# tczhangzhi/pytorch-distributed

Hardware: NVIDIA H100
Metric: ResNet-50 images/sec (device-timed, max over ranks) (higher is better)
Workload: dtype bf16; 1 GPU; model=resnet50, global_batch=256, image_size=224, parallelism=dp1, entry=distributed, comm=fused, nvls=False, channels_last=True, fused_bn=True, optimizer=fused, cuda_graph=True, l2_policy=inputs larger than L2 (4 x 38.5 MB bf16 batches + GBs of activations per step), overlap_optimizer=True, bucket_view=False, cudnn=deterministic

## Files before the change

### pytorch_distributed_b200/csrc/bindings.cpp

```cpp
#include <torch/extension.h>

#include "hvd_core.h"
#include "host.h"
#include "symm.h"

namespace py = pybind11;
using namespace ptd;

namespace {

at::Tensor arena_view(const std::shared_ptr<SymmArena>& a, int64_t rank, int64_t offset_bytes, int64_t numel, const std::string& dtype) {
  at::ScalarType st;
  if (dtype == "float32") st = at::kFloat;
  else if (dtype == "bfloat16") st = at::kBFloat16;
  else if (dtype == "float16") st = at::kHalf;
  else if (dtype == "int32") st = at::kInt;
  else if (dtype == "uint8") st = at::kByte;
  else throw std::runtime_error("unsupported arena view dtype " + dtype);
  const int64_t esz = (int64_t)c10::elementSize(st);
  TORCH_CHECK(offset_bytes >= 0 && offset_bytes + numel * esz <= a->bytes(), "arena view out of range");
  TORCH_CHECK(offset_bytes % esz == 0, "misaligned arena view");
  const int r = a->single_process() ? (int)rank : a->rank();
  void* p = reinterpret_cast<void*>(a->ptr(r) + offset_bytes);
  auto keep = a;
  return at::from_blob(p, {numel}, [keep](void*) {}, at::TensorOptions().dtype(st).device(at::kCUDA, (c10::DeviceIndex)a->device(r)));
}

}

PYBIND11_MODULE(TORCH_EXTENSION_NAME, m) {
  m.doc() = "pytorch_distributed_b200 native runtime (sm_90a)";
  m.attr("MAX_WORLD") = kMaxWorld;
  m.attr("MAX_BLOCKS") = kMaxBlocks;
  m.attr("MAX_CHANNELS") = kMaxChannels;
  m.attr("MAX_PTRS") = kMaxPtrs;
  m.attr("SIGNAL_PAD_BYTES") = (int64_t)sizeof(SignalPad);
  m.attr("SEG_BYTES") = (int64_t)sizeof(Seg);
  m.def("multicast_supported", &multicast_supported);

  py::class_<SymmArena, std::shared_ptr<SymmArena>>(m, "SymmArena")
      .def(py::init<int, int, int, int64_t>(), py::arg("device"), py::arg("rank"), py::arg("world"), py::arg("bytes"))
      .def_static("create_local", &SymmArena::create_local)
      .def_static("from_pointers", &SymmArena::from_pointers)
      .def("export_fd", &SymmArena::export_fd)
      .def("open_socket", &SymmArena::open_socket)
      .def("send_fd", &SymmArena::send_fd)
      .def("recv_fd", &SymmArena::recv_fd, py::call_guard<py::gil_scoped_release>())
      .def("map_peer", &SymmArena::map_peer)
      .def("mc_create", &SymmArena::mc_create)
      .def("mc_import", &SymmArena::mc_import)
      .def("mc_add_device", &SymmArena::mc_add_device)
      .def("mc_bind_and_map", &SymmArena::mc_bind_and_map)
      .def("disable_multicast", &SymmArena::disable_multicast)
      .def_property_readonly("rank", &SymmArena::rank)
      .def_property_readonly("world", &SymmArena::world)
      .def_property_readonly("bytes", &SymmArena::bytes)
      .def_property_readonly("mc_ptr", &SymmArena::mc_ptr)
      .def_property_readonly("multicast_candidate", &SymmArena::multicast_candidate)
      .def_property_readonly("has_multicast", &SymmArena::has_multicast)
      .def_property_readonly("mc_error", &SymmArena::mc_error)
      .def_property_readonly("single_process", &SymmArena::single_process)
      .def("ptr", &SymmArena::ptr)
      .def("device", &SymmArena::device, py::arg("r") = 0)
      .def("status", &SymmArena::status)
      .def("set_timeout_ms", &SymmArena::set_timeout_ms)
      .def("ll_seq_ptr", &SymmArena::ll_seq_ptr, py::arg("r") = 0)
      .def("view", [](std::shared_ptr<SymmArena> a, int64_t offset, int64_t numel, const std::string& dtype, int64_t rank) {
             return arena_view(a, rank, offset, numel, dtype);
           }, py::arg("offset_bytes"), py::arg("numel"), py::arg("dtype"), py::arg("rank") = 0)
      .def("launch_plan",
           [](std::shared_ptr<SymmArena> a, int channel, int as_rank, int kind, int wire_dtype, bool nvls, int grid, std::vector<at::Tensor> tensors,
              int64_t seg_begin_ptr, int64_t segs_ptr, int64_t data_off_bytes, int64_t block_elems, int64_t plan_calls_ptr, int64_t found_inf_ptr,
              double scale, bool writeback, int root, int flags, int64_t result_off_bytes) {
             launch_plan(a->ctx(channel, as_rank), kind, wire_dtype, nvls, grid, tensors, seg_begin_ptr, segs_ptr, data_off_bytes, block_elems,
                         plan_calls_ptr, found_inf_ptr, scale, writeback, root, flags, result_off_bytes);
           },
           py::arg("channel"), py::arg("as_rank"), py::arg("kind"), py::arg("wire_dtype"), py::arg("nvls"), py::arg("grid"), py::arg("tensors"),
           py::arg("seg_begin_ptr"), py::arg("segs_ptr"), py::arg("data_off_bytes"), py::arg("block_elems"), py::arg("plan_calls_ptr"),
           py::arg("found_inf_ptr"), py::arg("scale"), py::arg("writeback"), py::arg("root"), py::arg("flags") = 0,
           py::arg("result_off_bytes") = (int64_t)-1)
      .def("launch_barrier", [](std::shared_ptr<SymmArena> a, int channel) { launch_barrier(a->ctx(channel)); })
      .def("launch_metrics",
           [](std::shared_ptr<SymmArena> a, int channel, const at::Tensor& logits, const at::Tensor& target, c10::optional<at::Tensor> loss, at::Tensor out) {
             launch_metrics(a->ctx(channel), logits, target, loss, a->ll_seq_ptr(), out);
           })
      .def("launch_ll_allreduce", [](std::shared_ptr<SymmArena> a, int channel, const at::Tensor& in, at::Tensor out, double scale) {
        launch_ll_allreduce(a->ctx(channel), in, out, scale, a->ll_seq_ptr());
      });

  m.def("pack_pointers", &pack_pointers);
  m.def("fused_sgd_flat", &fused_sgd_flat, py::arg("grad"), py::arg("master"), py::arg("momentum"), py::arg("model_copy"), py::arg("hyper"),
        py::arg("found_inf"), py::arg("nesterov"), py::arg("first_step"));
  m.def("fused_sgd_multi", &fused_sgd_multi);
  m.def("multi_tensor_scale", &multi_tensor_scale);
  m.def("multi_tensor_axpby", &multi_tensor_axpby);
  m.def("amp_update_scale", &amp_update_scale);
  m.def("bn_act_forward", &bn_act_forward);
  m.def("bn_act_backward", &bn_act_backward);
  m.def("bn_act_backward2", &bn_act_backward2);
  m.def("stem_forward", &stem_forward);
  m.def("stem_forward_pre", &stem_forward_pre);
  m.def("stem_backward", &stem_backward);
  m.def("stem_im2col", &stem_im2col);
  m.def("conv1x1_bnstats", &conv1x1_bnstats);
  m.def("normalize_nhwc", &normalize_nhwc);
  m.def("resample_normalize", &resample_normalize, py::arg("arena"), py::arg("n"), py::arg("out_h"), py::arg("out_w"), py::arg("max_rows"),
        py::arg("a"), py::arg("b"), py::arg("out_dtype"), py::arg("channels_last"));
  m.def("p2p_copy_multi", &p2p_copy_multi);

  py::class_<FusionQueue, std::shared_ptr<FusionQueue>>(m, "FusionQueue")
      .def(py::init<int64_t, double, int64_t>(), py::arg("fusion_threshold_bytes"), py::arg("cycle_time_ms"), py::arg("cycle_bytes") = 0)
      .def("wait_idle", &FusionQueue::wait_idle, py::arg("timeout_ms"), py::call_guard<py::gil_scoped_release>())
      .def("wake", &FusionQueue::wake)
      .def("set_cycle_bytes", &FusionQueue::set_cycle_bytes)
      .def("cycle_bytes", &FusionQueue::cycle_bytes)
      .def("enable_timeline", &FusionQueue::enable_timeline)
      .def("timeline", &FusionQueue::timeline)
      .def("enqueue", &FusionQueue::enqueue, py::arg("name"), py::arg("nbytes"), py::arg("order_key"))
      .def("next_group", &FusionQueue::next_group, py::arg("timeout_ms"), py::call_guard<py::gil_scoped_release>())
      .def("flush", &FusionQueue::flush)
      .def("mark_done", &FusionQueue::mark_done)
      .def("wait", &FusionQueue::wait, py::arg("handle"), py::arg("timeout_ms"), py::call_guard<py::gil_scoped_release>())
      .def("pending", &FusionQueue::pending)
      .def("shutdown", &FusionQueue::shutdown)
      .def("stats", &FusionQueue::stats);
}
```

### pytorch_distributed_b200/csrc/gemm_bnstats.cu

```cuda
#include <ATen/cuda/CUDAContext.h>
#include <c10/cuda/CUDAGuard.h>
#include <cuda.h>
#include <torch/extension.h>

#include "common.cuh"
#include "host.h"

namespace ptd {

constexpr int kBlockM = 128;
constexpr int kBlockK = 64;
constexpr int kConsumerThreads = 256;
constexpr int kGemmThreads = kConsumerThreads + 32;

template <int BLOCK_N> struct GemmCfg {
  static constexpr int kStages = BLOCK_N == 256 ? 3 : 4;
  static constexpr int kABytes = kBlockM * kBlockK * 2;
  static constexpr int kBBytes = BLOCK_N * kBlockK * 2;
  static constexpr int kCBytes = kBlockM * BLOCK_N * 2;
  static constexpr int kStatFloats = 2 * 4 * 128;
  static constexpr int kSmem = 1024 + kStages * (kABytes + kBBytes) + kCBytes + kStatFloats * 4 + 2 * kStages * 8;
};

__device__ __forceinline__ uint32_t smem_u32(const void* p) { return (uint32_t)__cvta_generic_to_shared(p); }

__device__ __forceinline__ void mbar_init(uint64_t* bar, uint32_t count) {
  asm volatile("mbarrier.init.shared::cta.b64 [%0], %1;" ::"r"(smem_u32(bar)), "r"(count));
}
__device__ __forceinline__ void mbar_expect_tx(uint64_t* bar, uint32_t bytes) {
  asm volatile("mbarrier.arrive.expect_tx.shared::cta.b64 _, [%0], %1;" ::"r"(smem_u32(bar)), "r"(bytes) : "memory");
}
__device__ __forceinline__ void mbar_arrive(uint64_t* bar) {
  asm volatile("mbarrier.arrive.shared::cta.b64 _, [%0];" ::"r"(smem_u32(bar)) : "memory");
}
__device__ __forceinline__ void mbar_wait(uint64_t* bar, uint32_t parity) {
  const uint32_t addr = smem_u32(bar);
  uint32_t done, spins = 0;
  do {
    asm volatile("{\n\t.reg .pred p;\n\tmbarrier.try_wait.parity.shared::cta.b64 p, [%1], %2;\n\tselp.u32 %0, 1, 0, p;\n\t}"
                 : "=r"(done) : "r"(addr), "r"(parity) : "memory");
    if (!done && ++spins > (1u << 24)) __trap();
  } while (!done);
}
__device__ __forceinline__ void tma_load_2d(void* smem_dst, const CUtensorMap* map, uint64_t* bar, int c0, int c1) {
  asm volatile("cp.async.bulk.tensor.2d.shared::cluster.global.mbarrier::complete_tx::bytes [%0], [%1, {%3, %4}], [%2];"
               ::"r"(smem_u32(smem_dst)), "l"(map), "r"(smem_u32(bar)), "r"(c0), "r"(c1) : "memory");
}
__device__ __forceinline__ void named_barrier(int id, int threads) {
  asm volatile("bar.sync %0, %1;" ::"r"(id), "r"(threads) : "memory");
}

__device__ __forceinline__ uint64_t gmma_desc(const void* smem_tile) {
  const uint64_t addr = (uint64_t)(smem_u32(smem_tile) >> 4) & 0x3FFFull;
  return addr | (1ull << 16) | ((uint64_t)(1024 >> 4) << 32) | (1ull << 62);
}

#define PTD_F8(i) "+f"(d[i]), "+f"(d[i + 1]), "+f"(d[i + 2]), "+f"(d[i + 3]), "+f"(d[i + 4]), "+f"(d[i + 5]), "+f"(d[i + 6]), "+f"(d[i + 7])

__device__ __forceinline__ void wgmma_n64(float* d, uint64_t adesc, uint64_t bdesc, int accumulate) {
  asm volatile(
      "{\n\t.reg .pred p;\n\tsetp.ne.b32 p, %34, 0;\n\t"
      "wgmma.mma_async.sync.aligned.m64n64k16.f32.bf16.bf16 "
      "{%0, %1, %2, %3, %4, %5, %6, %7, %8, %9, %10, %11, %12, %13, %14, %15, "
      "%16, %17, %18, %19, %20, %21, %22, %23, %24, %25, %26, %27, %28, %29, %30, %31}, %32, %33, p, 1, 1, 0, 0;\n\t}"
      : PTD_F8(0), PTD_F8(8), PTD_F8(16), PTD_F8(24)
      : "l"(adesc), "l"(bdesc), "r"(accumulate));
}
__device__ __forceinline__ void wgmma_n128(float* d, uint64_t adesc, uint64_t bdesc, int accumulate) {
  asm volatile(
      "{\n\t.reg .pred p;\n\tsetp.ne.b32 p, %66, 0;\n\t"
      "wgmma.mma_async.sync.aligned.m64n128k16.f32.bf16.bf16 "
      "{%0, %1, %2, %3, %4, %5, %6, %7, %8, %9, %10, %11, %12, %13, %14, %15, "
      "%16, %17, %18, %19, %20, %21, %22, %23, %24, %25, %26, %27, %28, %29, %30, %31, "
      "%32, %33, %34, %35, %36, %37, %38, %39, %40, %41, %42, %43, %44, %45, %46, %47, "
      "%48, %49, %50, %51, %52, %53, %54, %55, %56, %57, %58, %59, %60, %61, %62, %63}, %64, %65, p, 1, 1, 0, 0;\n\t}"
      : PTD_F8(0), PTD_F8(8), PTD_F8(16), PTD_F8(24), PTD_F8(32), PTD_F8(40), PTD_F8(48), PTD_F8(56)
      : "l"(adesc), "l"(bdesc), "r"(accumulate));
}
#undef PTD_F8

template <int N> __device__ __forceinline__ void fence_regs(float (&d)[N]) {
#pragma unroll
  for (int i = 0; i < N; ++i) asm volatile("" : "+f"(d[i])::"memory");
}

template <int BLOCK_N>
__global__ void __launch_bounds__(kGemmThreads, 1) gemm_bnstats_kernel(const __grid_constant__ CUtensorMap tmap_a,
                                                                       const __grid_constant__ CUtensorMap tmap_b,
                                                                       const __grid_constant__ CUtensorMap tmap_c,
                                                                       float* __restrict__ part, int N, int K, int m_tiles,
                                                                       int n_tiles, int ctas_per_n) {
  using Cfg = GemmCfg<BLOCK_N>;
  constexpr int kStages = Cfg::kStages;
  constexpr int kInstN = BLOCK_N >= 128 ? 128 : 64;
  constexpr int kBoxes = BLOCK_N / 64;
  extern __shared__ uint8_t smem_raw[];
  uint8_t* smem = reinterpret_cast<uint8_t*>((reinterpret_cast<uintptr_t>(smem_raw) + 1023) & ~(uintptr_t)1023);
  uint8_t* smem_a = smem;
  uint8_t* smem_b = smem_a + kStages * Cfg::kABytes;
  uint8_t* smem_c = smem_b + kStages * Cfg::kBBytes;
  float* smem_stats = reinterpret_cast<float*>(smem_c + Cfg::kCBytes);
  uint64_t* full_bar = reinterpret_cast<uint64_t*>(smem_stats + Cfg::kStatFloats);
  uint64_t* empty_bar = full_bar + kStages;

  const int warp = threadIdx.x >> 5, lane = threadIdx.x & 31;
  const int n_tile = blockIdx.x % n_tiles;
  const int m_first = blockIdx.x / n_tiles;
  const int n0 = n_tile * BLOCK_N;
  const int num_kb = K / kBlockK;

  if (threadIdx.x == 0) {
    for (int s = 0; s < kStages; ++s) { mbar_init(&full_bar[s], 1); mbar_init(&empty_bar[s], kConsumerThreads / 32); }
    asm volatile("fence.mbarrier_init.release.cluster;" ::: "memory");
  }
  __syncthreads();

  if (warp == kConsumerThreads / 32) {
    if (lane == 0) {
      asm volatile("prefetch.tensormap [%0];" ::"l"(&tmap_a) : "memory");
      asm volatile("prefetch.tensormap [%0];" ::"l"(&tmap_b) : "memory");
      uint32_t it = 0;
      for (int mt = m_first; mt < m_tiles; mt += ctas_per_n) {
        for (int kb = 0; kb < num_kb; ++kb, ++it) {
          const int s = it % kStages;
          mbar_wait(&empty_bar[s], ((it / kStages) & 1) ^ 1);
          mbar_expect_tx(&full_bar[s], Cfg::kABytes + Cfg::kBBytes);
          tma_load_2d(smem_a + s * Cfg::kABytes, &tmap_a, &full_bar[s], kb * kBlockK, mt * kBlockM);
          tma_load_2d(smem_b + s * Cfg::kBBytes, &tmap_b, &full_bar[s], kb * kBlockK, n0);
        }
      }
    }
    return;
  }

  const int wg = warp >> 2, t = threadIdx.x & 127, w = warp & 3;
  uint8_t* stg = smem_c + wg * (Cfg::kCBytes / 2);
  float acc[BLOCK_N / 2] = {};
  const int r0 = 16 * w + (lane >> 2);
  constexpr int kPairs = BLOCK_N / 2, kParts = 128 / kPairs, kRows = 64 / kParts;
  const int p = t % kPairs, rpart = t / kPairs;
  const int p_box = p >> 5, p_gran = (p & 31) >> 2, p_byte = (p & 3) * 4;
  float s0 = 0.f, s1 = 0.f, q0 = 0.f, q1 = 0.f;

  uint32_t it = 0;
  for (int mt = m_first; mt < m_tiles; mt += ctas_per_n) {
    for (int kb = 0; kb < num_kb; ++kb, ++it) {
      const int s = it % kStages;
      mbar_wait(&full_bar[s], (it / kStages) & 1);
      const uint64_t adesc = gmma_desc(smem_a + s * Cfg::kABytes + wg * 64 * 128);
      const uint64_t bdesc = gmma_desc(smem_b + s * Cfg::kBBytes);
      fence_regs(acc);
      asm volatile("wgmma.fence.sync.aligned;" ::: "memory");
#pragma unroll
      for (int k = 0; k < kBlockK / 16; ++k) {
#pragma unroll
        for (int h = 0; h < BLOCK_N / kInstN; ++h) {
          if constexpr (kInstN == 128) wgmma_n128(acc + h * 64, adesc + 2 * k, bdesc + h * 8 * kInstN + 2 * k, (kb | k) != 0);
          else wgmma_n64(acc + h * 32, adesc + 2 * k, bdesc + h * 8 * kInstN + 2 * k, (kb | k) != 0);
        }
      }
      asm volatile("wgmma.commit_group.sync.aligned;" ::: "memory");
      asm volatile("wgmma.wait_group.sync.aligned 0;" ::: "memory");
      fence_regs(acc);
      if (lane == 0) mbar_arrive(&empty_bar[s]);
    }

    if (t == 0) asm volatile("cp.async.bulk.wait_group.read 0;" ::: "memory");
    named_barrier(1 + wg, 128);
#pragma unroll
    for (int j = 0; j < BLOCK_N / 8; ++j) {
      uint8_t* box = stg + (j >> 3) * 8192 + (lane & 3) * 4;
      const int g = j & 7;
      *reinterpret_cast<uint32_t*>(box + r0 * 128 + ((g ^ (r0 & 7)) << 4)) = Wire<__nv_bfloat16>::pack2(acc[4 * j], acc[4 * j + 1]);
      *reinterpret_cast<uint32_t*>(box + (r0 + 8) * 128 + ((g ^ (r0 & 7)) << 4)) =
          Wire<__nv_bfloat16>::pack2(acc[4 * j + 2], acc[4 * j + 3]);
    }
    asm volatile("fence.proxy.async.shared::cta;" ::: "memory");
    named_barrier(1 + wg, 128);
    if (t == 0) {
#pragma unroll
      for (int b = 0; b < kBoxes; ++b)
        asm volatile("cp.async.bulk.tensor.2d.global.shared::cta.bulk_group [%0, {%2, %3}], [%1];"
                     ::"l"(&tmap_c), "r"(smem_u32(stg + b * 8192)), "r"(n0 + b * 64), "r"(mt * kBlockM + wg * 64) : "memory");
      asm volatile("cp.async.bulk.commit_group;" ::: "memory");
    }
    const uint8_t* src = stg + p_box * 8192 + p_byte;
#pragma unroll 8
    for (int r = rpart * kRows; r < rpart * kRows + kRows; ++r) {
      const float2 f = Wire<__nv_bfloat16>::unpack2(*reinterpret_cast<const uint32_t*>(src + r * 128 + ((p_gran ^ (r & 7)) << 4)));
      s0 += f.x; q0 += f.x * f.x;
      s1 += f.y; q1 += f.y * f.y;
    }
  }
  if (t == 0) asm volatile("cp.async.bulk.wait_group 0;" ::: "memory");
  float* my = smem_stats + wg * 4 * 128 + t;
  my[0] = s0; my[128] = s1; my[256] = q0; my[384] = q1;
  named_barrier(3, kConsumerThreads);
  for (int i = threadIdx.x; i < 2 * BLOCK_N; i += kConsumerThreads) {
    const int half = i >= BLOCK_N, col = i - half * BLOCK_N;
    const int pair = col >> 1, which = half * 2 + (col & 1);
    float v = 0.f;
    for (int w2 = 0; w2 < 2; ++w2)
      for (int pt = 0; pt < kParts; ++pt) v += smem_stats[w2 * 4 * 128 + which * 128 + pt * kPairs + pair];
    part[(size_t)m_first * 2 * N + half * N + n0 + col] = v;
  }
}

typedef CUresult (*EncodeTiledFn)(CUtensorMap*, CUtensorMapDataType, cuuint32_t, void*, const cuuint64_t*, const cuuint64_t*, const cuuint32_t*,
                                  const cuuint32_t*, CUtensorMapInterleave, CUtensorMapSwizzle, CUtensorMapL2promotion, CUtensorMapFloatOOBfill);

static EncodeTiledFn encode_fn() {
  static EncodeTiledFn fn = nullptr;
  if (!fn) {
    void* p = nullptr;
    cudaDriverEntryPointQueryResult q;
    TORCH_CHECK(cudaGetDriverEntryPoint("cuTensorMapEncodeTiled", &p, cudaEnableDefault, &q) == cudaSuccess && p, "cuTensorMapEncodeTiled not found");
    fn = reinterpret_cast<EncodeTiledFn>(p);
  }
  return fn;
}

static CUtensorMap make_map(const void* ptr, int64_t rows, int64_t cols, int box_rows, CUtensorMapL2promotion promo) {
  CUtensorMap m;
  cuuint64_t dims[2] = {(cuuint64_t)cols, (cuuint64_t)rows};
  cuuint64_t strides[1] = {(cuuint64_t)cols * 2};
  cuuint32_t box[2] = {(cuuint32_t)kBlockK, (cuuint32_t)box_rows};
  cuuint32_t estr[2] = {1, 1};
  CUresult r = encode_fn()(&m, CU_TENSOR_MAP_DATA_TYPE_BFLOAT16, 2, const_cast<void*>(ptr), dims, strides, box, estr, CU_TENSOR_MAP_INTERLEAVE_NONE,
                           CU_TENSOR_MAP_SWIZZLE_128B, promo, CU_TENSOR_MAP_FLOAT_OOB_FILL_NONE);
  TORCH_CHECK(r == CUDA_SUCCESS, "cuTensorMapEncodeTiled failed: ", (int)r);
  return m;
}

template <int BLOCK_N>
static void launch_gemm(const at::Tensor& a, const at::Tensor& b, at::Tensor& c, at::Tensor& gsum, int M, int N, int K) {
  constexpr int smem = GemmCfg<BLOCK_N>::kSmem;
  static bool configured[64] = {};
  const int dev = a.get_device();
  if (!configured[dev & 63]) {
    C10_CUDA_CHECK(cudaFuncSetAttribute(gemm_bnstats_kernel<BLOCK_N>, cudaFuncAttributeMaxDynamicSharedMemorySize, smem));
    configured[dev & 63] = true;
  }
  const CUtensorMap ma = make_map(a.data_ptr(), M, K, kBlockM, CU_TENSOR_MAP_L2_PROMOTION_L2_256B);
  const CUtensorMap mb = make_map(b.data_ptr(), N, K, BLOCK_N, CU_TENSOR_MAP_L2_PROMOTION_L2_256B);
  const CUtensorMap mc = make_map(c.data_ptr(), M, N, 64, CU_TENSOR_MAP_L2_PROMOTION_NONE);
  const int m_tiles = (M + kBlockM - 1) / kBlockM, n_tiles = N / BLOCK_N;
  const int sms = at::cuda::getCurrentDeviceProperties()->multiProcessorCount;
  const int ctas_per_n = std::max(1, std::min(m_tiles, sms / n_tiles));
  const int grid = ctas_per_n * n_tiles;
  cudaStream_t st = at::cuda::getCurrentCUDAStream();
  at::Tensor part = at::empty({ctas_per_n, 2 * N}, gsum.options());
  gemm_bnstats_kernel<BLOCK_N><<<grid, kGemmThreads, smem, st>>>(ma, mb, mc, part.data_ptr<float>(), N, K, m_tiles, n_tiles, ctas_per_n);
  C10_CUDA_KERNEL_LAUNCH_CHECK();
  combine_partials(part.data_ptr<float>(), ctas_per_n, 2 * N, gsum.data_ptr<float>(), st);
}

at::Tensor conv1x1_bnstats(const at::Tensor& x, const at::Tensor& weight, at::Tensor gsum) {
  TORCH_CHECK(x.is_cuda() && x.dim() == 4 && x.scalar_type() == at::kBFloat16 && x.is_contiguous(at::MemoryFormat::ChannelsLast),
              "conv1x1_bnstats: x must be a channels_last bf16 CUDA tensor");
  TORCH_CHECK(weight.dim() == 4 && weight.size(2) == 1 && weight.size(3) == 1 && weight.scalar_type() == at::kBFloat16, "weight must be [N, K, 1, 1] bf16");
  const int64_t M64 = x.size(0) * x.size(2) * x.size(3);
  const int K = (int)x.size(1), N = (int)weight.size(0);
  TORCH_CHECK(weight.size(1) == K && K % kBlockK == 0 && N % 64 == 0 && M64 < (int64_t)1 << 31, "conv1x1_bnstats: unsupported shape");
  TORCH_CHECK(gsum.scalar_type() == at::kFloat && gsum.numel() >= 2 * N && gsum.is_contiguous());
  TORCH_CHECK((reinterpret_cast<uintptr_t>(x.data_ptr()) & 15) == 0, "x must be 16-byte aligned");
  c10::cuda::CUDAGuard guard(x.device());
  at::Tensor w2 = weight.reshape({N, K}).contiguous();
  at::Tensor y = at::empty({x.size(0), N, x.size(2), x.size(3)}, x.options().memory_format(at::MemoryFormat::ChannelsLast));
  const int M = (int)M64;
  static const int max_bn = getenv("PTD_GEMM_BLOCK_N") ? atoi(getenv("PTD_GEMM_BLOCK_N")) : 256;
  if (N % 256 == 0 && max_bn >= 256) launch_gemm<256>(x, w2, y, gsum, M, N, K);
  else if (N % 128 == 0 && max_bn >= 128) launch_gemm<128>(x, w2, y, gsum, M, N, K);
  else launch_gemm<64>(x, w2, y, gsum, M, N, K);
  return y;
}

}
```

### pytorch_distributed_b200/csrc/host.h

```cpp
#pragma once
#include <cuda_runtime_api.h>
#include <torch/extension.h>

#include <cstdint>
#include <string>
#include <vector>

#include "comm_types.h"

namespace ptd {

struct Seg {
  int32_t tensor;
  int32_t len;
  int64_t src_off;
  int64_t arena_off;
};
static_assert(sizeof(Seg) == 24, "Seg layout is mirrored by numpy in parallel/plan.py");

void launch_plan(const CommCtx& ctx, int kind, int wire_dtype, bool nvls, int grid, const std::vector<at::Tensor>& tensors,
                 int64_t seg_begin_ptr, int64_t segs_ptr, int64_t data_off_bytes, int64_t block_elems, int64_t plan_calls_ptr,
                 int64_t found_inf_ptr, double scale, bool writeback, int root, int flags = 0, int64_t result_off_bytes = -1);
at::Tensor pack_pointers(const std::vector<at::Tensor>& tensors);
void launch_barrier(const CommCtx& ctx);
void launch_metrics(const CommCtx& ctx, const at::Tensor& logits, const at::Tensor& target, const c10::optional<at::Tensor>& loss,
                    int64_t ll_seq_ptr, at::Tensor out);
void launch_ll_allreduce(const CommCtx& ctx, const at::Tensor& in, at::Tensor out, double scale, int64_t ll_seq_ptr);

void fused_sgd_flat(at::Tensor grad, at::Tensor master, at::Tensor momentum, c10::optional<at::Tensor> model_copy,
                    at::Tensor hyper, c10::optional<at::Tensor> found_inf, bool nesterov, bool first_step);
void fused_sgd_multi(std::vector<at::Tensor> grads, std::vector<at::Tensor> params, std::vector<at::Tensor> momenta,
                     std::vector<at::Tensor> model_copies, at::Tensor hyper, c10::optional<at::Tensor> found_inf, bool nesterov,
                     bool first_step);
void multi_tensor_scale(std::vector<at::Tensor> src, std::vector<at::Tensor> dst, double scale, at::Tensor found_inf);
void multi_tensor_axpby(std::vector<at::Tensor> x, std::vector<at::Tensor> y, std::vector<at::Tensor> out, double a, double b,
                        at::Tensor found_inf);
void amp_update_scale(at::Tensor scale, at::Tensor growth_tracker, at::Tensor found_inf, double growth, double backoff,
                      int64_t interval, at::Tensor hyper);

void combine_partials(const float* part, int nblocks, int n, float* gsum, cudaStream_t st);
std::vector<at::Tensor> bn_act_forward(const at::Tensor& x, const c10::optional<at::Tensor>& residual, const at::Tensor& weight,
                                       const at::Tensor& bias, at::Tensor running_mean, at::Tensor running_var,
                                       c10::optional<at::Tensor> num_batches_tracked, bool training, double momentum, double eps, bool relu,
                                       bool need_mask, at::Tensor work, bool stats_ready);
std::vector<at::Tensor> bn_act_backward(const at::Tensor& dy, const at::Tensor& x, const c10::optional<at::Tensor>& mask,
                                        const at::Tensor& weight, const at::Tensor& saved, bool relu, bool has_residual, at::Tensor work);
std::vector<at::Tensor> bn_act_backward2(const at::Tensor& dy_a, const at::Tensor& dy_b, const at::Tensor& x,
                                         const c10::optional<at::Tensor>& mask, const at::Tensor& weight, const at::Tensor& saved, bool relu,
                                         at::Tensor work);

std::vector<at::Tensor> stem_forward(const at::Tensor& x, const at::Tensor& weight, const at::Tensor& bias, at::Tensor running_mean,
                                     at::Tensor running_var, c10::optional<at::Tensor> num_batches_tracked, bool training, double momentum,
                                     double eps, bool need_code, at::Tensor work);
std::vector<at::Tensor> stem_forward_pre(const at::Tensor& x, const at::Tensor& weight, const at::Tensor& bias, at::Tensor running_mean,
                                         at::Tensor running_var, c10::optional<at::Tensor> num_batches_tracked, bool training, double momentum,
                                         double eps, bool need_code, at::Tensor work);
std::vector<at::Tensor> stem_backward(const at::Tensor& dp, const at::Tensor& x, const at::Tensor& code, const at::Tensor& weight,
                                      const at::Tensor& saved, at::Tensor work);

at::Tensor conv1x1_bnstats(const at::Tensor& x, const at::Tensor& weight, at::Tensor gsum);

at::Tensor stem_im2col(const at::Tensor& x);

at::Tensor normalize_nhwc(const at::Tensor& src, const at::Tensor& mean, const at::Tensor& std, int64_t out_dtype, bool channels_last);

void p2p_copy_multi(std::vector<at::Tensor> src, std::vector<at::Tensor> dst, int64_t run_device);

at::Tensor resample_normalize(const at::Tensor& arena, int64_t n, int64_t out_h, int64_t out_w, int64_t max_rows, const at::Tensor& a,
                              const at::Tensor& b, int64_t out_dtype, bool channels_last);

}
```

### pytorch_distributed_b200/csrc/stem_conv.cu

```cuda
#include <ATen/cuda/CUDAContext.h>
#include <c10/cuda/CUDAGuard.h>
#include <torch/extension.h>

#include "common.cuh"
#include "host.h"

namespace ptd {

constexpr int kStemK = 192;
constexpr int kStemRowK = 24;
constexpr int kStemGranules = kStemK / 8;

__device__ __forceinline__ V4 stem_granule_scalar(const unsigned short* __restrict__ row, int e0, int q, int row_elems) {
  unsigned short v[8];
#pragma unroll
  for (int j = 0; j < 8; ++j) {
    const int sc = q * 8 + j, e = e0 + j;
    v[j] = (sc < 21 && e >= 0 && e < row_elems) ? __ldg(row + e) : (unsigned short)0;
  }
  return V4{(uint32_t)v[0] | ((uint32_t)v[1] << 16), (uint32_t)v[2] | ((uint32_t)v[3] << 16), (uint32_t)v[4] | ((uint32_t)v[5] << 16),
            (uint32_t)v[6] | ((uint32_t)v[7] << 16)};
}

__global__ void __launch_bounds__(256) stem_im2col_scalar_kernel(const __nv_bfloat16* __restrict__ x, __nv_bfloat16* __restrict__ a, int H,
                                                                 int W, int OH, int OW) {
  const int g = blockIdx.y * blockDim.x + threadIdx.x;
  if (g >= OW * kStemGranules) return;
  const int orow = blockIdx.x;
  const int n = orow / OH, oh = orow - n * OH;
  const int ow = g / kStemGranules, gq = g - ow * kStemGranules;
  const int r = gq / 3, q = gq - 3 * r;
  const int row_elems = W * 3;
  V4 o{0u, 0u, 0u, 0u};
  const int ih = 2 * oh - 3 + r;
  if (r < 7 && ih >= 0 && ih < H) {
    const unsigned short* row = reinterpret_cast<const unsigned short*>(x) + ((int64_t)n * H + ih) * row_elems;
    o = stem_granule_scalar(row, (2 * ow - 3) * 3 + q * 8, q, row_elems);
  }
  st_v4(a + ((int64_t)orow * OW * kStemGranules + g) * 8, o);
}

constexpr int kStemPad = 16;

__global__ void __launch_bounds__(256) stem_im2col_kernel(const __nv_bfloat16* __restrict__ x, __nv_bfloat16* __restrict__ a, int H, int W,
                                                          int OH, int OW) {
  extern __shared__ __align__(16) unsigned char stem_smem[];
  const int row_elems = W * 3;
  const int srow = row_elems + 2 * kStemPad;
  unsigned short* sm = reinterpret_cast<unsigned short*>(stem_smem);
  const int orow = blockIdx.x;
  const int n = orow / OH, oh = orow - n * OH;
  const int vec_per_row = srow / 8;
  for (int v = threadIdx.x; v < 7 * vec_per_row; v += blockDim.x) {
    const int r = v / vec_per_row, c = v - r * vec_per_row;
    const int ih = 2 * oh - 3 + r;
    const int e = c * 8 - kStemPad;
    V4 val{0u, 0u, 0u, 0u};
    if (ih >= 0 && ih < H && e >= 0 && e < row_elems)
      val = ld_stream(reinterpret_cast<const unsigned short*>(x) + ((int64_t)n * H + ih) * row_elems + e);
    *reinterpret_cast<V4*>(sm + r * srow + c * 8) = val;
  }
  __syncthreads();
  const int total = OW * kStemGranules;
  __nv_bfloat16* out = a + (int64_t)orow * total * 8;
  for (int g = threadIdx.x; g < total; g += blockDim.x) {
    const int ow = g / kStemGranules, gq = g - ow * kStemGranules;
    const int r = gq / 3, q = gq - 3 * r;
    V4 o{0u, 0u, 0u, 0u};
    if (r < 7) {
      const int e0 = (2 * ow - 3) * 3 + q * 8 + kStemPad;
      const uint32_t* w = reinterpret_cast<const uint32_t*>(sm + r * srow + (e0 - 1));
      const uint32_t w0 = w[0], w1 = w[1], w2 = w[2], w3 = w[3], w4 = w[4];
      o.x = __byte_perm(w0, w1, 0x5432);
      o.y = __byte_perm(w1, w2, 0x5432);
      o.z = __byte_perm(w2, w3, 0x5432);
      o.w = __byte_perm(w3, w4, 0x5432);
      if (q == 2) {
        o.z &= 0x0000FFFFu;
        o.w = 0u;
      }
    }
    st_v4(out + (int64_t)g * 8, o);
  }
}

at::Tensor stem_im2col(const at::Tensor& x) {
  TORCH_CHECK(x.is_cuda() && x.dim() == 4 && x.size(1) == 3 && x.scalar_type() == at::kBFloat16 &&
                  x.is_contiguous(at::MemoryFormat::ChannelsLast),
              "stem_im2col: x must be a [N, 3, H, W] channels_last bf16 CUDA tensor");
  const int64_t N = x.size(0);
  const int H = (int)x.size(2), W = (int)x.size(3);
  const int OH = (H + 6 - 7) / 2 + 1, OW = (W + 6 - 7) / 2 + 1;
  TORCH_CHECK(H >= 7 && W >= 7 && (int64_t)W * 3 < (1 << 30), "stem_im2col: unsupported image size");
  c10::cuda::CUDAGuard guard(x.device());
  at::Tensor a = at::empty({N, OH, OW, kStemK}, x.options());
  TORCH_CHECK(N * OH < ((int64_t)1 << 31) && (int64_t)OW * kStemGranules < (1 << 24), "stem_im2col: too many output rows");
  const __nv_bfloat16* xp = reinterpret_cast<const __nv_bfloat16*>(x.data_ptr());
  __nv_bfloat16* ap = reinterpret_cast<__nv_bfloat16*>(a.data_ptr());
  cudaStream_t st = at::cuda::getCurrentCUDAStream();
  const int64_t row_elems = (int64_t)W * 3;
  const size_t smem = (size_t)7 * (row_elems + 2 * kStemPad) * 2;
  if (row_elems % 8 == 0 && (reinterpret_cast<uintptr_t>(x.data_ptr()) & 15) == 0 && smem <= 96 * 1024) {
    if (smem > 48 * 1024) {
      static bool attr_set[64] = {};
      const int dev = x.get_device();
      if (dev >= 0 && dev < 64 && !attr_set[dev]) {
        C10_CUDA_CHECK(cudaFuncSetAttribute(stem_im2col_kernel, cudaFuncAttributeMaxDynamicSharedMemorySize, 96 * 1024));
        attr_set[dev] = true;
      }
    }
    stem_im2col_kernel<<<(unsigned)(N * OH), 256, smem, st>>>(xp, ap, H, W, OH, OW);
  } else {
    dim3 grid((unsigned)(N * OH), (unsigned)((OW * kStemGranules + 255) / 256));
    stem_im2col_scalar_kernel<<<grid, 256, 0, st>>>(xp, ap, H, W, OH, OW);
  }
  C10_CUDA_KERNEL_LAUNCH_CHECK();
  return a.permute({0, 3, 1, 2});
}

}
```

### pytorch_distributed_b200/ops/stem_conv.py

```python
from __future__ import annotations

import torch
import torch.nn.functional as F

from .bn_act import workspace
from .stem import _StemFn, bn_relu_maxpool, can_fuse_stem

K_PAD = 192
ROW_K = 24


def pack_stem_weight(weight: torch.Tensor) -> torch.Tensor:
    co = weight.size(0)
    w = weight.permute(0, 2, 3, 1).reshape(co, 7, 21)
    w = F.pad(w, (0, ROW_K - 21)).reshape(co, 7 * ROW_K)
    return F.pad(w, (0, K_PAD - 7 * ROW_K)).contiguous()


def unpack_stem_weight(packed: torch.Tensor, like: torch.Tensor) -> torch.Tensor:
    co = packed.size(0)
    w = packed[:, : 7 * ROW_K].reshape(co, 7, ROW_K)[:, :, :21].reshape(co, 7, 7, 3).permute(0, 3, 1, 2)
    out = torch.empty_like(like)
    out.copy_(w)
    return out


def im2col_reference(x: torch.Tensor) -> torch.Tensor:
    n, c, h, w = x.shape
    assert c == 3
    oh, ow = (h + 6 - 7) // 2 + 1, (w + 6 - 7) // 2 + 1
    cols = F.unfold(x.float(), kernel_size=7, padding=3, stride=2)
    cols = cols.reshape(n, 3, 7, 7, oh * ow).permute(0, 4, 2, 3, 1).reshape(n, oh * ow, 7, 21)
    a = F.pad(cols, (0, ROW_K - 21)).reshape(n, oh * ow, 7 * ROW_K)
    a = F.pad(a, (0, K_PAD - 7 * ROW_K)).to(x.dtype)
    return a.reshape(n, oh, ow, K_PAD).permute(0, 3, 1, 2)


def can_use_stem_gemm(x: torch.Tensor, conv) -> bool:
    w = conv.weight
    return (x.is_cuda and x.dtype == torch.bfloat16 and w.dtype == torch.bfloat16 and x.dim() == 4 and x.size(1) == 3
            and not x.requires_grad and conv.kernel_size == (7, 7) and conv.stride == (2, 2) and conv.padding == (3, 3)
            and conv.dilation == (1, 1) and conv.groups == 1 and conv.bias is None and w.size(0) % 64 == 0
            and x.is_contiguous(memory_format=torch.channels_last) and x.size(2) >= 7 and x.size(3) >= 7)


class _StemConvFn(torch.autograd.Function):

    @staticmethod
    def forward(ctx, x, weight, stats, emulate=False):
        packed = pack_stem_weight(weight)
        if emulate:
            a = im2col_reference(x).contiguous(memory_format=torch.channels_last)
            rows = a.permute(0, 2, 3, 1).reshape(-1, K_PAD)
            y2 = (rows.float() @ packed.float().t()).to(x.dtype)
            if stats is not None:
                stats[: y2.size(1)] += y2.float().sum(0)
                stats[y2.size(1): 2 * y2.size(1)] += (y2.float() ** 2).sum(0)
            y = y2.reshape(a.size(0), a.size(2), a.size(3), -1).permute(0, 3, 1, 2)
        else:
            from .. import _ext
            C = _ext.lib()
            _ext.note_launch(3)
            a = C.stem_im2col(x)
            y = C.conv1x1_bnstats(a, packed.view(packed.size(0), K_PAD, 1, 1), stats)
        ctx.save_for_backward(a, weight)
        return y

    @staticmethod
    def backward(ctx, dy):
        a, weight = ctx.saved_tensors
        co = weight.size(0)
        dy2 = dy.permute(0, 2, 3, 1).reshape(-1, co)
        rows = a.permute(0, 2, 3, 1).reshape(-1, K_PAD)
        if dy2.dtype != rows.dtype:
            dy2 = dy2.to(rows.dtype)
        if rows.is_cuda and rows.dtype != torch.float32:
            dwp = torch.mm(dy2.t(), rows, out_dtype=torch.float32)
        else:
            dwp = dy2.float().t() @ rows.float()
        return None, unpack_stem_weight(dwp, weight), None, None


class _StemPreFn(torch.autograd.Function):

    @staticmethod
    def forward(ctx, x, weight, bias, running_mean, running_var, nbt, momentum, eps, need_grad, work, gen):
        from .. import _ext
        nc = x.size(1)
        _ext.note_launch(1)
        y, saved, code = _ext.lib().stem_forward_pre(x, weight, bias, running_mean, running_var, nbt, True, momentum, eps, need_grad,
                                                     work[: 2 * nc])
        ctx.work = work[2 * nc:]
        ctx.gen, ctx.ws = gen, workspace(x.device)
        if need_grad:
            ctx.save_for_backward(x, code, weight, saved)
        return y

    @staticmethod
    def backward(ctx, dy):
        return _StemFn.backward(ctx, dy) + (None,)


def stem_conv_bn_relu_maxpool(x, conv, bn, emulate: bool = False):
    nc = conv.weight.size(0)
    momentum = 0.1 if bn.momentum is None else float(bn.momentum)
    nbt = bn.num_batches_tracked if (bn.training and bn.track_running_stats) else None
    if emulate:
        y = _StemConvFn.apply(x, conv.weight, None, True)
        return bn_relu_maxpool(y, bn.weight, bn.bias, bn.running_mean, bn.running_var, training=True, momentum=momentum, eps=bn.eps,
                               fused=False, num_batches_tracked=nbt)
    ws = workspace(x.device)
    work, gen = ws.take(4 * nc)
    y = _StemConvFn.apply(x, conv.weight, work[: 2 * nc], False)
    if not can_fuse_stem(y, bn.weight, bn.running_mean):
        raise RuntimeError("stem GEMM output does not fit the fused stem tail")
    need_grad = torch.is_grad_enabled() and (y.requires_grad or bn.weight.requires_grad)
    return _StemPreFn.apply(y, bn.weight, bn.bias, bn.running_mean, bn.running_var, nbt, momentum, float(bn.eps), need_grad, work, gen)
```

Before: 6038 images/s.

## Fuse stem im2col into the GEMM+BN-stats kernel with an on-chip producer warpgroup

Adds a stem variant of the TMA GEMM+bnstats kernel. A 128-thread producer warpgroup bulk-copies input image rows into shared memory, builds the im2col K-blocks on-chip for the wgmma consumers, and keeps the small weight matrix resident. The im2col matrix is still written to global memory via TMA stores, because backward needs it for dW, but the separate im2col kernel launch and its read back from HBM are removed. The cost is a more complex producer/consumer pipeline with extra shared-memory row buffers, which could lower occupancy or stall if the on-chip im2col build is slow.

```diff
diff --git a/pytorch_distributed_b200/csrc/bindings.cpp b/pytorch_distributed_b200/csrc/bindings.cpp
--- a/pytorch_distributed_b200/csrc/bindings.cpp
+++ b/pytorch_distributed_b200/csrc/bindings.cpp
@@ -103,6 +103,8 @@
   m.def("stem_backward", &stem_backward);
   m.def("stem_im2col", &stem_im2col);
   m.def("conv1x1_bnstats", &conv1x1_bnstats);
+  m.def("stem_implicit_supported", &stem_implicit_supported);
+  m.def("stem_conv_bnstats", &stem_conv_bnstats);
   m.def("normalize_nhwc", &normalize_nhwc);
   m.def("resample_normalize", &resample_normalize, py::arg("arena"), py::arg("n"), py::arg("out_h"), py::arg("out_w"), py::arg("max_rows"),
         py::arg("a"), py::arg("b"), py::arg("out_dtype"), py::arg("channels_last"));
diff --git a/pytorch_distributed_b200/csrc/gemm_bnstats.cu b/pytorch_distributed_b200/csrc/gemm_bnstats.cu
--- a/pytorch_distributed_b200/csrc/gemm_bnstats.cu
+++ b/pytorch_distributed_b200/csrc/gemm_bnstats.cu
@@ -5,6 +5,7 @@
 
 #include "common.cuh"
 #include "host.h"
+#include "stem_layout.cuh"
 
 namespace ptd {
 
@@ -29,6 +30,9 @@
 }
 __device__ __forceinline__ void mbar_expect_tx(uint64_t* bar, uint32_t bytes) {
   asm volatile("mbarrier.arrive.expect_tx.shared::cta.b64 _, [%0], %1;" ::"r"(smem_u32(bar)), "r"(bytes) : "memory");
+}
+__device__ __forceinline__ void mbar_expect_tx_only(uint64_t* bar, uint32_t bytes) {
+  asm volatile("mbarrier.expect_tx.relaxed.cta.shared::cta.b64 [%0], %1;" ::"r"(smem_u32(bar)), "r"(bytes) : "memory");
 }
 __device__ __forceinline__ void mbar_arrive(uint64_t* bar) {
   asm volatile("mbarrier.arrive.shared::cta.b64 _, [%0];" ::"r"(smem_u32(bar)) : "memory");
@@ -84,12 +88,107 @@
   for (int i = 0; i < N; ++i) asm volatile("" : "+f"(d[i])::"memory");
 }
 
-template <int BLOCK_N>
-__global__ void __launch_bounds__(kGemmThreads, 1) gemm_bnstats_kernel(const __grid_constant__ CUtensorMap tmap_a,
-                                                                       const __grid_constant__ CUtensorMap tmap_b,
-                                                                       const __grid_constant__ CUtensorMap tmap_c,
-                                                                       float* __restrict__ part, int N, int K, int m_tiles,
-                                                                       int n_tiles, int ctas_per_n) {
+struct TmaA {
+  struct Args {};
+  static constexpr int kThreads = kGemmThreads;
+  static constexpr int kFullArrivals = 1;
+  static constexpr bool kResidentB = false;
+};
+
+constexpr int kMaxRowBufs = 4;
+struct StemGeom {
+  const __nv_bfloat16* x;
+  int H, W, OH, OW, M, srow, max_rows, nbuf;
+};
+
+struct StemA {
+  using Args = StemGeom;
+  static constexpr int kThreads = kConsumerThreads + 128;
+  static constexpr int kFullArrivals = 128;
+  static constexpr bool kResidentB = true;
+};
+constexpr int kStemProducerBar = 4;
+
+__device__ __forceinline__ void stem_stage_rows(const StemGeom& g, int mt, unsigned short* rows, uint64_t* bar, int lane) {
+  const int m0 = mt * kBlockM, m1 = min(m0 + kBlockM, g.M) - 1;
+  const int orow0 = m0 / g.OW, slots = (m1 / g.OW - orow0 + 1) * 7;
+  const int n0 = orow0 / g.OH, oh0 = orow0 - n0 * g.OH;
+  const uint32_t row_bytes = g.W * 3 * 2;
+  for (int base = 0; base < slots; base += 32) {
+    const int sl = base + lane, j = sl / 7, r = sl - 7 * j;
+    int n = n0, oh = oh0 + j;
+    while (oh >= g.OH) { oh -= g.OH; ++n; }
+    const int ih = 2 * oh - 3 + r;
+    const bool live = sl < slots && ih >= 0 && ih < g.H;
+    const uint32_t mask = __ballot_sync(0xffffffffu, live);
+    if (base == 0) {
+      int total = __popc(mask);
+      for (int b2 = 32; b2 < slots; b2 += 32) {
+        const int s2 = b2 + lane, j2 = s2 / 7, r2 = s2 - 7 * j2;
+        int oh2 = oh0 + j2;
+        while (oh2 >= g.OH) oh2 -= g.OH;
+        const int ih2 = 2 * oh2 - 3 + r2;
+        total += __popc(__ballot_sync(0xffffffffu, s2 < slots && ih2 >= 0 && ih2 < g.H));
+      }
+      if (lane == 0) mbar_expect_tx(bar, total * row_bytes);
+      __syncwarp();
+    }
+    if (live)
+      asm volatile("cp.async.bulk.shared::cluster.global.mbarrier::complete_tx::bytes [%0], [%1], %2, [%3];"
+                   ::"r"(smem_u32(rows + sl * g.srow + kStemPad)), "l"(g.x + ((int64_t)n * g.H + ih) * g.W * 3), "r"(row_bytes),
+                   "r"(smem_u32(bar)) : "memory");
+  }
+}
+
+struct StemPixel {
+  const unsigned short* pix;
+  int r_lo, r_hi;
+};
+
+__device__ __forceinline__ void stem_build_kblock(const StemPixel& p, int srow, uint8_t* stage, int t, int kb) {
+  uint8_t* row = stage + t * 128;
+#pragma unroll
+  for (int gi = 0; gi < 8; ++gi) {
+    const int gq = kb * 8 + gi, r = gq / 3, q = gq - 3 * r;
+    V4 o{0u, 0u, 0u, 0u};
+    if (r < 7 && r >= p.r_lo && r <= p.r_hi) o = stem_granule(reinterpret_cast<const uint32_t*>(p.pix + r * srow + q * 8), q);
+    *reinterpret_cast<V4*>(row + ((gi ^ (t & 7)) << 4)) = o;
+  }
+}
+
+template <class Emit>
+__device__ __forceinline__ void stem_producer_loop(const StemGeom& g, unsigned short* rows, uint64_t* rows_bar, int first, int end, int step,
+                                                   int t, Emit&& emit) {
+  const int buf = 7 * g.max_rows * g.srow;
+  for (int sl = t; sl < g.nbuf * 7 * g.max_rows; sl += 128) {
+    unsigned short* s = rows + sl * g.srow;
+    *reinterpret_cast<V4*>(s) = V4{0u, 0u, 0u, 0u};
+    *reinterpret_cast<V4*>(s + 8) = V4{0u, 0u, 0u, 0u};
+    *reinterpret_cast<V4*>(s + g.srow - 16) = V4{0u, 0u, 0u, 0u};
+    *reinterpret_cast<V4*>(s + g.srow - 8) = V4{0u, 0u, 0u, 0u};
+  }
+  if (t < 32)
+    for (int b = 0; b < g.nbuf - 1 && first + b * step < end; ++b) stem_stage_rows(g, first + b * step, rows + b * buf, &rows_bar[b], t);
+  int i = 0;
+  for (int mt = first; mt < end; mt += step, ++i) {
+    const int b = i % g.nbuf, ahead = mt + (g.nbuf - 1) * step, bn = (i + g.nbuf - 1) % g.nbuf;
+    named_barrier(kStemProducerBar, 128);
+    if (t < 32 && ahead < end) stem_stage_rows(g, ahead, rows + bn * buf, &rows_bar[bn], t);
+    mbar_wait(&rows_bar[b], (i / g.nbuf) & 1);
+    const int m = mt * kBlockM + t;
+    const int orow = m / g.OW, ow = m - orow * g.OW, j = orow - mt * kBlockM / g.OW, oh = orow % g.OH;
+    StemPixel p{rows + b * buf + j * 7 * g.srow + (2 * ow - 3) * 3 + kStemPad - 1, max(0, 3 - 2 * oh), min(6, g.H + 2 - 2 * oh)};
+    if (m >= g.M) p.r_lo = 7;
+    emit(mt, p);
+  }
+}
+
+template <int BLOCK_N, class P>
+__global__ void __launch_bounds__(P::kThreads, 1) gemm_bnstats_kernel(const __grid_constant__ CUtensorMap tmap_a,
+                                                                      const __grid_constant__ CUtensorMap tmap_b,
+                                                                      const __grid_constant__ CUtensorMap tmap_c,
+                                                                      float* __restrict__ part, int N, int K, int m_tiles,
+                                                                      int n_tiles, int ctas_per_n, const typename P::Args pa) {
   using Cfg = GemmCfg<BLOCK_N>;
   constexpr int kStages = Cfg::kStages;
   constexpr int kInstN = BLOCK_N >= 128 ? 128 : 64;
@@ -110,27 +209,61 @@
   const int num_kb = K / kBlockK;
 
   if (threadIdx.x == 0) {
-    for (int s = 0; s < kStages; ++s) { mbar_init(&full_bar[s], 1); mbar_init(&empty_bar[s], kConsumerThreads / 32); }
+    for (int s = 0; s < kStages; ++s) { mbar_init(&full_bar[s], P::kFullArrivals); mbar_init(&empty_bar[s], kConsumerThreads / 32); }
+    if constexpr (P::kResidentB) for (int b = 0; b < pa.nbuf; ++b) mbar_init(&empty_bar[kStages + b], 1);
     asm volatile("fence.mbarrier_init.release.cluster;" ::: "memory");
   }
   __syncthreads();
 
-  if (warp == kConsumerThreads / 32) {
-    if (lane == 0) {
-      asm volatile("prefetch.tensormap [%0];" ::"l"(&tmap_a) : "memory");
-      asm volatile("prefetch.tensormap [%0];" ::"l"(&tmap_b) : "memory");
+  if constexpr (P::kResidentB) {
+    if (warp >= kConsumerThreads / 32) {
+      const int t = threadIdx.x - kConsumerThreads;
+      if (t == 0) {
+        asm volatile("prefetch.tensormap [%0];" ::"l"(&tmap_b) : "memory");
+        mbar_expect_tx_only(&full_bar[0], kStemK / kBlockK * Cfg::kBBytes);
+        for (int kb = 0; kb < kStemK / kBlockK; ++kb) tma_load_2d(smem_b + kb * Cfg::kBBytes, &tmap_b, &full_bar[0], kb * kBlockK, n0);
+      }
       uint32_t it = 0;
-      for (int mt = m_first; mt < m_tiles; mt += ctas_per_n) {
-        for (int kb = 0; kb < num_kb; ++kb, ++it) {
-          const int s = it % kStages;
-          mbar_wait(&empty_bar[s], ((it / kStages) & 1) ^ 1);
-          mbar_expect_tx(&full_bar[s], Cfg::kABytes + Cfg::kBBytes);
-          tma_load_2d(smem_a + s * Cfg::kABytes, &tmap_a, &full_bar[s], kb * kBlockK, mt * kBlockM);
-          tma_load_2d(smem_b + s * Cfg::kBBytes, &tmap_b, &full_bar[s], kb * kBlockK, n0);
+      stem_producer_loop(pa, reinterpret_cast<unsigned short*>(empty_bar + kStages + kMaxRowBufs), empty_bar + kStages, m_first, m_tiles, ctas_per_n, t,
+                         [&](int mt, const StemPixel& px) {
+#pragma unroll
+                           for (int kb = 0; kb < kStemK / kBlockK; ++kb, ++it) {
+                             const int s = it % kStages;
+                             mbar_wait(&empty_bar[s], ((it / kStages) & 1) ^ 1);
+                             stem_build_kblock(px, pa.srow, smem_a + s * Cfg::kABytes, t, kb);
+                             asm volatile("fence.proxy.async.shared::cta;" ::: "memory");
+                             if (t == 0) asm volatile("cp.async.bulk.wait_group.read %0;" ::"n"(kStages - 2) : "memory");
+                             named_barrier(kStemProducerBar, 128);
+                             mbar_arrive(&full_bar[s]);
+                             if (t == 0) {
+                               asm volatile("cp.async.bulk.tensor.2d.global.shared::cta.bulk_group [%0, {%2, %3}], [%1];"
+                                            ::"l"(&tmap_a), "r"(smem_u32(smem_a + s * Cfg::kABytes)), "r"(kb * kBlockK), "r"(mt * kBlockM)
+                                            : "memory");
+                               asm volatile("cp.async.bulk.commit_group;" ::: "memory");
+                             }
+                           }
+                         });
+      if (t == 0) asm volatile("cp.async.bulk.wait_group 0;" ::: "memory");
+      return;
+    }
+  } else {
+    if (warp == kConsumerThreads / 32) {
+      if (lane == 0) {
+        asm volatile("prefetch.tensormap [%0];" ::"l"(&tmap_a) : "memory");
+        asm volatile("prefetch.tensormap [%0];" ::"l"(&tmap_b) : "memory");
+        uint32_t it = 0;
+        for (int mt = m_first; mt < m_tiles; mt += ctas_per_n) {
+          for (int kb = 0; kb < num_kb; ++kb, ++it) {
+            const int s = it % kStages;
+            mbar_wait(&empty_bar[s], ((it / kStages) & 1) ^ 1);
+            mbar_expect_tx(&full_bar[s], Cfg::kABytes + Cfg::kBBytes);
+            tma_load_2d(smem_a + s * Cfg::kABytes, &tmap_a, &full_bar[s], kb * kBlockK, mt * kBlockM);
+            tma_load_2d(smem_b + s * Cfg::kBBytes, &tmap_b, &full_bar[s], kb * kBlockK, n0);
+          }
         }
       }
-    }
-    return;
+      return;
+    }
   }
 
   const int wg = warp >> 2, t = threadIdx.x & 127, w = warp & 3;
@@ -148,7 +281,7 @@
       const int s = it % kStages;
       mbar_wait(&full_bar[s], (it / kStages) & 1);
       const uint64_t adesc = gmma_desc(smem_a + s * Cfg::kABytes + wg * 64 * 128);
-      const uint64_t bdesc = gmma_desc(smem_b + s * Cfg::kBBytes);
+      const uint64_t bdesc = gmma_desc(smem_b + (P::kResidentB ? kb : s) * Cfg::kBBytes);
       fence_regs(acc);
       asm volatile("wgmma.fence.sync.aligned;" ::: "memory");
 #pragma unroll
@@ -238,7 +371,7 @@
   static bool configured[64] = {};
   const int dev = a.get_device();
   if (!configured[dev & 63]) {
-    C10_CUDA_CHECK(cudaFuncSetAttribute(gemm_bnstats_kernel<BLOCK_N>, cudaFuncAttributeMaxDynamicSharedMemorySize, smem));
+    C10_CUDA_CHECK(cudaFuncSetAttribute(gemm_bnstats_kernel<BLOCK_N, TmaA>, cudaFuncAttributeMaxDynamicSharedMemorySize, smem));
     configured[dev & 63] = true;
   }
   const CUtensorMap ma = make_map(a.data_ptr(), M, K, kBlockM, CU_TENSOR_MAP_L2_PROMOTION_L2_256B);
@@ -250,7 +383,8 @@
   const int grid = ctas_per_n * n_tiles;
   cudaStream_t st = at::cuda::getCurrentCUDAStream();
   at::Tensor part = at::empty({ctas_per_n, 2 * N}, gsum.options());
-  gemm_bnstats_kernel<BLOCK_N><<<grid, kGemmThreads, smem, st>>>(ma, mb, mc, part.data_ptr<float>(), N, K, m_tiles, n_tiles, ctas_per_n);
+  gemm_bnstats_kernel<BLOCK_N, TmaA><<<grid, kGemmThreads, smem, st>>>(ma, mb, mc, part.data_ptr<float>(), N, K, m_tiles, n_tiles, ctas_per_n,
+                                                                       TmaA::Args{});
   C10_CUDA_KERNEL_LAUNCH_CHECK();
   combine_partials(part.data_ptr<float>(), ctas_per_n, 2 * N, gsum.data_ptr<float>(), st);
 }
@@ -275,4 +409,72 @@
   return y;
 }
 
-}
+constexpr int kStemCout = 64;
+
+static int stem_row_bufs(const StemGeom& g, size_t smem, size_t limit, size_t* bytes) {
+  const size_t buf = (size_t)7 * g.max_rows * g.srow * 2;
+  const size_t room = limit > smem + 8 * kMaxRowBufs ? limit - smem - 8 * kMaxRowBufs : 0;
+  const int n = (int)std::min<size_t>(kMaxRowBufs, room / buf);
+  *bytes = 8 * kMaxRowBufs + n * buf;
+  return n >= 2 ? n : 0;
+}
+
+static bool stem_implicit_geom(const at::Tensor& x, StemGeom& g, size_t& rows_bytes) {
+  if (!(x.is_cuda() && x.dim() == 4 && x.size(1) == 3 && x.scalar_type() == at::kBFloat16 && x.is_contiguous(at::MemoryFormat::ChannelsLast)))
+    return false;
+  const int64_t N = x.size(0), H = x.size(2), W = x.size(3);
+  if (H < 7 || W < 7 || (W * 3) % 8 != 0 || W * 3 >= (1 << 20) || (reinterpret_cast<uintptr_t>(x.data_ptr()) & 15) != 0) return false;
+  const int64_t OH = (H - 1) / 2 + 1, OW = (W - 1) / 2 + 1, M = N * OH * OW;
+  if (M == 0 || M >= ((int64_t)1 << 31) - kBlockM) return false;
+  g.x = reinterpret_cast<const __nv_bfloat16*>(x.data_ptr());
+  g.H = (int)H; g.W = (int)W; g.OH = (int)OH; g.OW = (int)OW; g.M = (int)M;
+  g.srow = (int)W * 3 + 2 * kStemPad;
+  g.max_rows = (int)((kBlockM - 1 + OW - 1) / OW) + 1;
+  const size_t limit = at::cuda::getDeviceProperties(x.get_device())->sharedMemPerBlockOptin;
+  g.nbuf = stem_row_bufs(g, GemmCfg<64>::kSmem, limit, &rows_bytes);
+  return g.nbuf > 0;
+}
+
+bool stem_implicit_supported(const at::Tensor& x, int64_t c_out) {
+  StemGeom g;
+  size_t rows_bytes;
+  return c_out == kStemCout && stem_implicit_geom(x, g, rows_bytes);
+}
+
+template <class Kernel> static void allow_max_smem(Kernel k, int dev, bool (&configured)[64]) {
+  if (!configured[dev & 63]) {
+    C10_CUDA_CHECK(cudaFuncSetAttribute(k, cudaFuncAttributeMaxDynamicSharedMemorySize,
+                                        (int)at::cuda::getDeviceProperties(dev)->sharedMemPerBlockOptin));
+    configured[dev & 63] = true;
+  }
+}
+
+std::vector<at::Tensor> stem_conv_bnstats(const at::Tensor& x, const at::Tensor& packed_w, at::Tensor gsum) {
+  c10::cuda::CUDAGuard guard(x.device());
+  StemGeom g;
+  size_t rows_bytes;
+  TORCH_CHECK(stem_implicit_geom(x, g, rows_bytes), "stem_conv_bnstats: unsupported input (stem_implicit_supported is false)");
+  TORCH_CHECK(packed_w.is_cuda() && packed_w.dim() == 2 && packed_w.size(0) == kStemCout && packed_w.size(1) == kStemK &&
+                  packed_w.scalar_type() == at::kBFloat16, "stem_conv_bnstats: packed_w must be [64, 192] bf16");
+  TORCH_CHECK(gsum.scalar_type() == at::kFloat && gsum.numel() >= 2 * kStemCout && gsum.is_contiguous());
+  at::Tensor w = packed_w.contiguous();
+  at::Tensor y = at::empty({x.size(0), kStemCout, g.OH, g.OW}, x.options().memory_format(at::MemoryFormat::ChannelsLast));
+  at::Tensor a = at::empty({x.size(0), g.OH, g.OW, kStemK}, x.options());
+  static bool configured[64] = {};
+  allow_max_smem(gemm_bnstats_kernel<64, StemA>, x.get_device(), configured);
+  const CUtensorMap mb = make_map(w.data_ptr(), kStemCout, kStemK, 64, CU_TENSOR_MAP_L2_PROMOTION_L2_256B);
+  const CUtensorMap mc = make_map(y.data_ptr(), g.M, kStemCout, 64, CU_TENSOR_MAP_L2_PROMOTION_NONE);
+  const CUtensorMap ma = make_map(a.data_ptr(), g.M, kStemK, kBlockM, CU_TENSOR_MAP_L2_PROMOTION_NONE);
+  const int m_tiles = (g.M + kBlockM - 1) / kBlockM;
+  const int sms = at::cuda::getCurrentDeviceProperties()->multiProcessorCount;
+  const int ctas = std::max(1, std::min(m_tiles, sms));
+  cudaStream_t st = at::cuda::getCurrentCUDAStream();
+  at::Tensor part = at::empty({ctas, 2 * kStemCout}, gsum.options());
+  gemm_bnstats_kernel<64, StemA><<<ctas, StemA::kThreads, GemmCfg<64>::kSmem + rows_bytes, st>>>(
+      ma, mb, mc, part.data_ptr<float>(), kStemCout, kStemK, m_tiles, 1, ctas, g);
+  C10_CUDA_KERNEL_LAUNCH_CHECK();
+  combine_partials(part.data_ptr<float>(), ctas, 2 * kStemCout, gsum.data_ptr<float>(), st);
+  return {y, a.permute({0, 3, 1, 2})};
+}
+
+}
diff --git a/pytorch_distributed_b200/csrc/host.h b/pytorch_distributed_b200/csrc/host.h
--- a/pytorch_distributed_b200/csrc/host.h
+++ b/pytorch_distributed_b200/csrc/host.h
@@ -59,6 +59,8 @@
                                       const at::Tensor& saved, at::Tensor work);
 
 at::Tensor conv1x1_bnstats(const at::Tensor& x, const at::Tensor& weight, at::Tensor gsum);
+bool stem_implicit_supported(const at::Tensor& x, int64_t c_out);
+std::vector<at::Tensor> stem_conv_bnstats(const at::Tensor& x, const at::Tensor& packed_w, at::Tensor gsum);
 
 at::Tensor stem_im2col(const at::Tensor& x);
 
diff --git a/pytorch_distributed_b200/csrc/stem_conv.cu b/pytorch_distributed_b200/csrc/stem_conv.cu
--- a/pytorch_distributed_b200/csrc/stem_conv.cu
+++ b/pytorch_distributed_b200/csrc/stem_conv.cu
@@ -4,12 +4,9 @@
 
 #include "common.cuh"
 #include "host.h"
+#include "stem_layout.cuh"
 
 namespace ptd {
-
-constexpr int kStemK = 192;
-constexpr int kStemRowK = 24;
-constexpr int kStemGranules = kStemK / 8;
 
 __device__ __forceinline__ V4 stem_granule_scalar(const unsigned short* __restrict__ row, int e0, int q, int row_elems) {
   unsigned short v[8];
@@ -40,8 +37,6 @@
   st_v4(a + ((int64_t)orow * OW * kStemGranules + g) * 8, o);
 }
 
-constexpr int kStemPad = 16;
-
 __global__ void __launch_bounds__(256) stem_im2col_kernel(const __nv_bfloat16* __restrict__ x, __nv_bfloat16* __restrict__ a, int H, int W,
                                                           int OH, int OW) {
   extern __shared__ __align__(16) unsigned char stem_smem[];
@@ -69,16 +64,7 @@
     V4 o{0u, 0u, 0u, 0u};
     if (r < 7) {
       const int e0 = (2 * ow - 3) * 3 + q * 8 + kStemPad;
-      const uint32_t* w = reinterpret_cast<const uint32_t*>(sm + r * srow + (e0 - 1));
-      const uint32_t w0 = w[0], w1 = w[1], w2 = w[2], w3 = w[3], w4 = w[4];
-      o.x = __byte_perm(w0, w1, 0x5432);
-      o.y = __byte_perm(w1, w2, 0x5432);
-      o.z = __byte_perm(w2, w3, 0x5432);
-      o.w = __byte_perm(w3, w4, 0x5432);
-      if (q == 2) {
-        o.z &= 0x0000FFFFu;
-        o.w = 0u;
-      }
+      o = stem_granule(reinterpret_cast<const uint32_t*>(sm + r * srow + (e0 - 1)), q);
     }
     st_v4(out + (int64_t)g * 8, o);
   }
diff --git a/pytorch_distributed_b200/csrc/stem_layout.cuh b/pytorch_distributed_b200/csrc/stem_layout.cuh
--- /dev/null
+++ b/pytorch_distributed_b200/csrc/stem_layout.cuh
@@ -0,0 +1,27 @@
+#pragma once
+#include <stdint.h>
+
+#include "common.cuh"
+
+namespace ptd {
+
+constexpr int kStemK = 192;
+constexpr int kStemRowK = 24;
+constexpr int kStemGranules = kStemK / 8;
+constexpr int kStemPad = 16;
+
+__device__ __forceinline__ V4 stem_granule(const uint32_t* w, int q) {
+  const uint32_t w0 = w[0], w1 = w[1], w2 = w[2], w3 = w[3], w4 = w[4];
+  V4 o;
+  o.x = __byte_perm(w0, w1, 0x5432);
+  o.y = __byte_perm(w1, w2, 0x5432);
+  o.z = __byte_perm(w2, w3, 0x5432);
+  o.w = __byte_perm(w3, w4, 0x5432);
+  if (q == 2) {
+    o.z &= 0x0000FFFFu;
+    o.w = 0u;
+  }
+  return o;
+}
+
+}
diff --git a/pytorch_distributed_b200/ops/stem_conv.py b/pytorch_distributed_b200/ops/stem_conv.py
--- a/pytorch_distributed_b200/ops/stem_conv.py
+++ b/pytorch_distributed_b200/ops/stem_conv.py
@@ -60,9 +60,13 @@
         else:
             from .. import _ext
             C = _ext.lib()
-            _ext.note_launch(3)
-            a = C.stem_im2col(x)
-            y = C.conv1x1_bnstats(a, packed.view(packed.size(0), K_PAD, 1, 1), stats)
+            if C.stem_implicit_supported(x, packed.size(0)):
+                _ext.note_launch(2)
+                y, a = C.stem_conv_bnstats(x, packed, stats)
+            else:
+                _ext.note_launch(3)
+                a = C.stem_im2col(x)
+                y = C.conv1x1_bnstats(a, packed.view(packed.size(0), K_PAD, 1, 1), stats)
         ctx.save_for_backward(a, weight)
         return y
 
```

Result: no change. 6089 images/s (median of 6 runs) (+0.8%).
